# rccohn/AMPIS

Hardware: AMD Instinct MI355X
Metric: images/sec Mask R-CNN R50-FPN @1024x1024 inference (higher is better)
Workload: dtype f32 (convs: f16x3 split-operand MFMA -- 22-bit operands, exact products, fp32 accumulate); 1 GPU; BASELINE configs[1]: R50-FPN inference, batch=8 synthetic 1024x1024 micrographs per GPU, K=2, 1000 proposals/img, TEST.DETECTIONS_PER_IMAGE=200, seeded random-init weights, outputs on the host: boxes, scores, classes and every mask as its COCO compressed-RLE counts string (encoded on the device); batch_per_gpu=8, global_batch=8, parallelism=image-parallel replicas x1, no data-path collective

## Files before the change

ampis_amd/csrc/conv.hip:

```cpp
#include "common.h"
#include <type_traits>

namespace {

typedef float f32x4 __attribute__((ext_vector_type(4)));
typedef float f32x16 __attribute__((ext_vector_type(16)));
typedef _Float16 f16x8 __attribute__((ext_vector_type(8)));
typedef _Float16 f16x2 __attribute__((ext_vector_type(2)));
typedef _Float16 f16x4 __attribute__((ext_vector_type(4)));
typedef unsigned int u32x4 __attribute__((ext_vector_type(4)));
constexpr float LO_SCALE = 2048.0f;

constexpr int BK = 32;
constexpr int LDS_LD = 36;

struct ConvArgs {
    const float* x;
    const float* w;
    const float* scale;
    const float* shift;
    const float* res;
    const float* mask;
    float* y;
    int B, H, W, Cin;
// ... 169 lines not shown
            } else {
#pragma unroll
                for (int q = 0; q < 4; ++q)
                    if (n + q < a.Cout) o[q] = a.mask[yoff[it] + q] > 0.f ? o[q] : 0.f;
            }
        }
        if (vec) {
            *reinterpret_cast<f32x4*>(a.y + yoff[it]) = o;
        } else {
#pragma unroll
            for (int q = 0; q < 4; ++q)
                if (n + q < a.Cout) a.y[yoff[it] + q] = o[q];
        }
    }
}

template <int MB, int NB>
struct F16x3Frags {
    f16x8 ah[MB], al[MB], bh[NB], bl[NB];
};
template <int MB, int NB>
__device__ __forceinline__ void f16x3_load16(const float* As, const float* Bs, int fo_hi, int fo_lo, F16x3Frags<MB, NB>& f) {
#pragma unroll
    for (int i = 0; i < MB; ++i) {
        f.ah[i] = *reinterpret_cast<const f16x8*>(As + i * 16 * BK + fo_hi);
        f.al[i] = *reinterpret_cast<const f16x8*>(As + i * 16 * BK + fo_lo);
    }
#pragma unroll
    for (int j = 0; j < NB; ++j) {
        f.bh[j] = *reinterpret_cast<const f16x8*>(Bs + j * 16 * BK + fo_hi);
        f.bl[j] = *reinterpret_cast<const f16x8*>(Bs + j * 16 * BK + fo_lo);
    }
}
template <int MB, int NB, bool SWAP = false>
__device__ __forceinline__ void f16x3_mfma16(const F16x3Frags<MB, NB>& f, f32x4 (&acc)[MB][NB], f32x4 (&acx)[MB][NB]) {
#pragma unroll
    for (int i = 0; i < MB; ++i) {
        if (SWAP) {
#pragma unroll
            for (int j = 0; j < NB; ++j) acx[i][j] = __builtin_amdgcn_mfma_f32_16x16x32_f16(f.bh[j], f.al[i], acx[i][j], 0, 0, 0);
#pragma unroll
            for (int j = 0; j < NB; ++j) acx[i][j] = __builtin_amdgcn_mfma_f32_16x16x32_f16(f.bl[j], f.ah[i], acx[i][j], 0, 0, 0);
#pragma unroll
            for (int j = 0; j < NB; ++j) acc[i][j] = __builtin_amdgcn_mfma_f32_16x16x32_f16(f.bh[j], f.ah[i], acc[i][j], 0, 0, 0);
        } else {
#pragma unroll
            for (int j = 0; j < NB; ++j) acx[i][j] = __builtin_amdgcn_mfma_f32_16x16x32_f16(f.al[i], f.bh[j], acx[i][j], 0, 0, 0);
#pragma unroll
            for (int j = 0; j < NB; ++j) acx[i][j] = __builtin_amdgcn_mfma_f32_16x16x32_f16(f.ah[i], f.bl[j], acx[i][j], 0, 0, 0);
#pragma unroll
            for (int j = 0; j < NB; ++j) acc[i][j] = __builtin_amdgcn_mfma_f32_16x16x32_f16(f.ah[i], f.bh[j], acc[i][j], 0, 0, 0);
        }
    }
}
template <int MB, int NB>
__device__ __forceinline__ void f16x3_step16(const float* As, const float* Bs, int fo_hi, int fo_lo, f32x4 (&acc)[MB][NB], f32x4 (&acx)[MB][NB]) {
    F16x3Frags<MB, NB> f;
    f16x3_load16<MB, NB>(As, Bs, fo_hi, fo_lo, f);
    f16x3_mfma16<MB, NB>(f, acc, acx);
}

template <int WTM, int WTN, bool SPATIAL, bool CHECK>
__device__ __forceinline__ void conv_epilogue_rows(const ConvArgs& a, float* stage, int lane, int mw0, int nw0);
template <int WTM, int WTN, bool SPATIAL, bool CHECK>
__device__ __forceinline__ void conv_epilogue_rows8(const ConvArgs& a, float* stage, int lane, int mw0, int nw0);

template <int WTM, int WTN, int MT, int NT, bool SPATIAL, bool CHECK = false>
__device__ __forceinline__ void conv_epilogue_fast(const ConvArgs& a, f32x16 (&acc)[MT][NT], float* lds, int wave, int lane,
                                                   int mw0, int nw0) {
    const int l31 = lane & 31, lh = lane >> 5;
    constexpr int SLD = WTN + 4;
    float* stage = lds + wave * (WTM * SLD);
#pragma unroll
    for (int i = 0; i < MT; ++i)
#pragma unroll
        for (int j = 0; j < NT; ++j)
#pragma unroll
            for (int e = 0; e < 16; ++e)
                stage[(i * 32 + (e & 3) + 8 * (e >> 2) + 4 * lh) * SLD + j * 32 + l31] = acc[i][j][e];
    if (a.y_split && !a.mask && a.out_mode == 0) conv_epilogue_rows8<WTM, WTN, SPATIAL, CHECK>(a, stage, lane, mw0, nw0);
    else conv_epilogue_rows<WTM, WTN, SPATIAL, CHECK>(a, stage, lane, mw0, nw0);
}

template <int WTM, int WTN, int MT, int NT, bool SPATIAL, bool CHECK = false>
__device__ __forceinline__ void conv_epilogue_fast16(const ConvArgs& a, f32x4 (&acc)[MT][NT], float* lds, int wave, int lane,
                                                     int mw0, int nw0) {
    const int l15 = lane & 15, lq = lane >> 4;
    constexpr int SLD = WTN + 4;
    float* stage = lds + wave * (WTM * SLD);
#pragma unroll
    for (int i = 0; i < MT; ++i)
#pragma unroll
        for (int j = 0; j < NT; ++j)
#pragma unroll
            for (int e = 0; e < 4; ++e)
                stage[(i * 16 + 4 * lq + e) * SLD + j * 16 + l15] = acc[i][j][e];
    if (a.y_split && !a.mask && a.out_mode == 0) conv_epilogue_rows8<WTM, WTN, SPATIAL, CHECK>(a, stage, lane, mw0, nw0);
    else conv_epilogue_rows<WTM, WTN, SPATIAL, CHECK>(a, stage, lane, mw0, nw0);
}

template <int WTM, int WTN, bool SPATIAL, bool CHECK>
__device__ __forceinline__ void conv_epilogue_rows8(const ConvArgs& a, float* stage, int lane, int mw0, int nw0) {
    constexpr int SLD = WTN + 4;
    constexpr int L8R = WTN / 8;
    constexpr int RPI = 64 / L8R;
    constexpr int NIT = WTM / RPI;
// ... 1072 lines not shown
            STAMP_T(t2);
            f16x3_load16<MB, NB>(As0 + cur * TILE_FLOATS, Bs0 + cur * TILE_FLOATS, fo16_hi, fo16_lo, fr);
            __builtin_amdgcn_sched_barrier(0);
            STAMP_T(t3);
            if (step + 2 < a.nsteps) stage(nxt);
            __builtin_amdgcn_sched_barrier(0);
            STAMP_T(t4);
            STAMP_ADD(0, t0, t1); STAMP_ADD(3, t1, t2); STAMP_ADD(2, t2, t3); STAMP_ADD(1, t3, t4);
            advance();
        }
        f16x3_mfma16<MB, NB, true>(fr, acc, acx);
    }
#ifdef AMP_STAMP
    if (wave == 0 && lane == 0) {
        atomicAdd(&g_stamp_clk[0], __builtin_amdgcn_s_memtime() - st_mt0);
        atomicAdd(&g_stamp_clk[1], __builtin_amdgcn_s_memrealtime() - st_rt0);
    }
    st_acc[4] = clock64() - st_begin;
    st_acc[5] = st_begin - st_entry;
    const long long st_loop_end = clock64();
#endif
    __syncthreads();
#ifdef AMP_STAMP
    st_acc[7] = clock64() - st_loop_end;
#endif
    const bool scaled_in = a.out_scale != 1.0f;

#pragma unroll
    for (int i = 0; i < MB; ++i)
#pragma unroll
        for (int j = 0; j < NB; ++j)
#pragma unroll
            for (int e = 0; e < 4; ++e) {
                acc[i][j][e] = __fadd_rn(acc[i][j][e], __fmul_rn(acx[i][j][e], 1.0f / LO_SCALE));
                if (scaled_in) acc[i][j][e] *= a.out_scale;
            }
    if constexpr (BM == 128 && BN == 256 && EPI == 3) {
        if (NBP == 1 && a.out_mode == 3) conv_epilogue_predict(a, acc, lds, wave, lane, m0, n0, ppf);
        else conv_epilogue_rpn<NBP>(a, acc, lds, wave, lane, m0, n0);
        return;
    }
    if (a.y_split && (!a.mask || a.mask_split) && (a.out_mode == 0 || (EPI == 2 && a.out_mode == 1 && !a.mask && a.res_mode == 0)) && (a.res_mode == 0 || a.res_split) && a.direct_epi)
        conv_epilogue_direct<EPI == 2, true>(a, acc, lane, m0 + wm * WTM, n0 + wn * WTN);
    else
        conv_epilogue_swapped<WTM, WTN, EPI == 2, true>(a, acc, lds, wave, lane, m0 + wm * WTM, n0 + wn * WTN);
#ifdef AMP_STAMP
    st_acc[6] = clock64() - st_loop_end;
    if (lane == 0)
        for (int q = 0; q < 8; ++q) atomicAdd(&g_stamp[wave * 8 + q], (unsigned long long)st_acc[q]);
#endif
}


__global__ __launch_bounds__(512, 1) void mask_tail_kernel(const ConvArgs a, const unsigned int x_bytes, const unsigned int w_bytes) {
    constexpr int BM = 128, BN = 256, NW = 8, GA = 2, GB = 4, NDMA = GA + GB, NTAP = 4;
    constexpr int TILE_FLOATS = (BM + BN) * BK;
    __shared__ __attribute__((aligned(16))) float lds[3 * TILE_FLOATS + 4 * BM + 2 * 256 + 4 + NTAP * BN];
    float* red = lds + 3 * TILE_FLOATS;
    float* wps = red + 4 * BM;
    float* pbs = wps + 2 * 256;
    float* dbias = pbs + 4;
    const int tid = threadIdx.x, lane = tid & 63;
    const int wave = __builtin_amdgcn_readfirstlane(tid >> 6);
    const int wm = wave >> 2, wn = wave & 3;
    const int l15 = lane & 15, lq = lane >> 4;
    const int m0 = amp::xcd_remap(blockIdx.x, a.nblk) * BM;
    const __amdgpu_buffer_rsrc_t rsrc_x = __builtin_amdgcn_make_buffer_rsrc(const_cast<float*>(a.x), 0, x_bytes, 0x00020000);
    const __amdgpu_buffer_rsrc_t rsrc_w = __builtin_amdgcn_make_buffer_rsrc(const_cast<float*>(a.w), 0, w_bytes, 0x00020000);
    const int srow = lane >> 3, spos = lane & 7;
    unsigned int a_voff[GA], b_voff[GB];
#pragma unroll
    for (int g = 0; g < GA; ++g) {
        const int r = wave * (BM / NW) + 8 * g + srow;
        const int m = m0 + r;
        a_voff[g] = (m < a.M) ? (unsigned int)(((size_t)m * a.Cin + 4 * (spos ^ ((r >> 1) & 7))) * 4) : OOB_VOFF;
    }
#pragma unroll
    for (int g = 0; g < GB; ++g) {
        const int r = wave * (BN / NW) + 8 * g + srow;
        const int n = (r & ~63) + swap_channel(r & 63);
        b_voff[g] = (unsigned int)(((size_t)n * a.K + 4 * (spos ^ ((r >> 1) & 7))) * 4);
    }
    const int csteps = a.Cin / BK;
    const int total = NTAP * csteps;
    const int tap_bytes = BN * a.K * 4;
    int s_cs = 0, s_tap = 0;
    auto stage = [&](int buf) {
        float* As = lds + buf * TILE_FLOATS;
        float* Bs = As + BM * BK;
        const int a_soff = s_cs * (BK * 4);
        const int b_soff = s_tap * tap_bytes + s_cs * (BK * 4);
#pragma unroll
        for (int g = 0; g < GA; ++g)
            __builtin_amdgcn_raw_ptr_buffer_load_lds(rsrc_x, (__attribute__((address_space(3))) void*)(As + (wave * (BM / NW) + 8 * g) * BK), 16, (int)a_voff[g], a_soff, 0, 0);
#pragma unroll
        for (int g = 0; g < GB; ++g)
            __builtin_amdgcn_raw_ptr_buffer_load_lds(rsrc_w, (__attribute__((address_space(3))) void*)(Bs + (wave * (BN / NW) + 8 * g) * BK), 16, (int)b_voff[g], b_soff, 0, 0);
        if (++s_cs == csteps) { s_cs = 0; ++s_tap; }
    };
    f32x4 acc[4][4], acx[4][4];
    auto zero_acc = [&]() {
#pragma unroll
        for (int i = 0; i < 4; ++i)
#pragma unroll
            for (int j = 0; j < 4; ++j)
#pragma unroll
                for (int e = 0; e < 4; ++e) { acc[i][j][e] = 0.f; acx[i][j][e] = 0.f; }
    };
    zero_acc();
    const int fo16_hi = 4 * (lq ^ (l15 >> 1)), fo16_lo = 4 * ((4 + lq) ^ (l15 >> 1));
    stage(0);
    stage(1);
    const int mw0 = m0 + wm * 64;
    const unsigned int b_first = fastdiv(min((unsigned int)m0, (unsigned int)(a.M - 1)), a.div_howo_mul, a.div_howo_shr);
    {
        const unsigned int b_last = fastdiv(min((unsigned int)(m0 + BM - 1), (unsigned int)(a.M - 1)), a.div_howo_mul, a.div_howo_shr);
        const int slot = tid >> 8, col = tid & 255;
        int c = a.pred_cls[slot ? b_last : b_first];
        c = (c >= 0 && c < a.pred_K) ? c : 0;
        wps[tid] = a.pred_w[(size_t)c * 256 + col];
        if (col == 0) pbs[slot] = a.pred_b[c];
        dbias[tid] = a.shift ? a.shift[tid] : 0.f;
        dbias[512 + tid] = a.shift ? a.shift[512 + tid] : 0.f;
    }
    bool bad = false;
    auto partial_sums = [&](int tap) {
        f32x4 bias[4];
#pragma unroll
        for (int j = 0; j < 4; ++j) bias[j] = *reinterpret_cast<const f32x4*>(dbias + tap * BN + wn * 64 + 32 * (j >> 1) + 8 * lq + 4 * (j & 1));
#pragma unroll
        for (int i = 0; i < 4; ++i) {
            const unsigned int m = min((unsigned int)(mw0 + i * 16 + l15), (unsigned int)(a.M - 1));
            const unsigned int b = fastdiv(m, a.div_howo_mul, a.div_howo_shr);
            const float* wrow = wps + ((b == b_first) ? 0 : 256) + wn * 64 + 8 * lq;
            float sj[4];
#pragma unroll
            for (int j = 0; j < 4; ++j) {
                const f32x4 wp = *reinterpret_cast<const f32x4*>(wrow + 32 * (j >> 1) + 4 * (j & 1));
                float sg = 0.f;
#pragma unroll
                for (int e = 0; e < 4; ++e) {
                    const float v = __fadd_rn(acc[i][j][e], __fmul_rn(acx[i][j][e], 1.0f / LO_SCALE));
                    bad = bad || !(fabsf(v) <= 3.0e38f);
                    const float o = fmaxf(__fadd_rn(v, bias[j][e]), 0.f);
                    sg = __fadd_rn(sg, __fmul_rn(o, wp[e]));
                }
                sj[j] = sg;
            }
            float u0 = __fadd_rn(sj[0], sj[2]), u1 = __fadd_rn(sj[1], sj[3]);
            u0 = __fadd_rn(u0, __shfl_xor(u0, 32)); u1 = __fadd_rn(u1, __shfl_xor(u1, 32));
            u0 = __fadd_rn(u0, __shfl_xor(u0, 16)); u1 = __fadd_rn(u1, __shfl_xor(u1, 16));
            const float sres = __fadd_rn(u0, u1);
            if (lq == 0) red[wn * BM + wm * 64 + i * 16 + l15] = sres;
        }
    };
    auto finish_rows = [&](int tap) {
        const int rl = wm * 64 + lane;
        const int m = m0 + rl;
        if (m < a.M) {
            const unsigned int b = fastdiv((unsigned int)m, a.div_howo_mul, a.div_howo_shr);
            const unsigned int rem = (unsigned int)m - b * (unsigned int)(a.Ho * a.Wo);
            const unsigned int oy = fastdiv(rem, a.div_wo_mul, a.div_wo_shr);
            const unsigned int ox = rem - oy * (unsigned int)a.Wo;
            float x = __fadd_rn(__fadd_rn(__fadd_rn(red[rl], red[BM + rl]), red[2 * BM + rl]), red[3 * BM + rl]);
            x = __fadd_rn(x, pbs[(b == b_first) ? 0 : 1]);
            const float p = __fdiv_rn(1.0f, __fadd_rn(1.0f, expf(-x)));
            a.prob[((size_t)b * 2 * a.Ho + 2 * oy + (tap >> 1)) * (2 * a.Wo) + 2 * ox + (tap & 1)] = p;
        }
    };
    int cur = 0, nxt = 2, c_cs = 0, c_tap = 0;
    auto open_step = [&](int step) {
        if (step + 1 < total) __builtin_amdgcn_s_waitcnt(0x0070 | NDMA);
        else __builtin_amdgcn_s_waitcnt(0x0070);
        asm volatile("" ::: "memory");
        __builtin_amdgcn_s_barrier();
        asm volatile("" ::: "memory");
    };
    auto advance = [&]() {
        cur = (cur == 2) ? 0 : cur + 1;
        nxt = (nxt == 2) ? 0 : nxt + 1;
        if (++c_cs == csteps) { c_cs = 0; ++c_tap; }
    };
    F16x3Frags<4, 4> fr;
    const float* As0 = lds + (wm * 64 + l15) * BK;
    const float* Bs0 = lds + BM * BK + (wn * 64 + l15) * BK;
    if (wave < NW / 2) {
        for (int step = 0; step < total; ++step) {
            open_step(step);
            if (c_cs == 0 && c_tap > 0 && wn == 0) finish_rows(c_tap - 1);
            f16x3_load16<4, 4>(As0 + cur * TILE_FLOATS, Bs0 + cur * TILE_FLOATS, fo16_hi, fo16_lo, fr);
            __builtin_amdgcn_sched_barrier(0);
            if (step + 2 < total) stage(nxt);
            __builtin_amdgcn_sched_barrier(0);
            __builtin_amdgcn_s_barrier();
            __builtin_amdgcn_s_setprio(1);
            f16x3_mfma16<4, 4, true>(fr, acc, acx);
            __builtin_amdgcn_s_setprio(0);
            __builtin_amdgcn_sched_barrier(0);
            if (c_cs == csteps - 1) { partial_sums(c_tap); zero_acc(); }
            advance();
        }
    } else {
        for (int step = 0; step < total; ++step) {
            open_step(step);
            __builtin_amdgcn_s_setprio(1);
            if (step > 0) f16x3_mfma16<4, 4, true>(fr, acc, acx);
            __builtin_amdgcn_s_setprio(0);
            __builtin_amdgcn_sched_barrier(0);
            const bool tap_done = c_cs == 0 && c_tap > 0;
            if (tap_done) { partial_sums(c_tap - 1); zero_acc(); __builtin_amdgcn_s_waitcnt(0xc07f); }
            __builtin_amdgcn_s_barrier();
            if (tap_done && wn == 0) finish_rows(c_tap - 1);
            f16x3_load16<4, 4>(As0 + cur * TILE_FLOATS, Bs0 + cur * TILE_FLOATS, fo16_hi, fo16_lo, fr);
            __builtin_amdgcn_sched_barrier(0);
            if (step + 2 < total) stage(nxt);
            __builtin_amdgcn_sched_barrier(0);
            advance();
        }
        f16x3_mfma16<4, 4, true>(fr, acc, acx);
        partial_sums(NTAP - 1);
    }
    __syncthreads();
    if (wn == 0) finish_rows(NTAP - 1);
    if (bad) atomicOr(a.range_flag, 1);
}

template <bool SPATIAL>
__global__ __launch_bounds__(512, 1) void conv1x1_nloop_kernel(const ConvArgs a, const unsigned int x_bytes, const unsigned int w_bytes, const int NT) {
    constexpr int BM = 128, BN = 256, NW = 8, GA = 2, GB = 4, NDMA = GA + GB, NST = 16;
    constexpr int TILE_FLOATS = (BM + BN) * BK;
    constexpr int NT_MAX = 8;
    __shared__ __attribute__((aligned(16))) float lds[3 * TILE_FLOATS + 2 * NT_MAX * BN];
    float* lsc = lds + 3 * TILE_FLOATS;
    float* lsh = lsc + NT_MAX * BN;
    const int tid = threadIdx.x, lane = tid & 63;
    const int wave = __builtin_amdgcn_readfirstlane(tid >> 6);
    const int wm = wave >> 2, wn = wave & 3;
    const int l15 = lane & 15, lq = lane >> 4;
    const int ngrp = a.ntn / NT;
    const int wg = amp::xcd_remap(blockIdx.x, a.nblk);
    const int grp = wg % ngrp;
    const int m0 = (wg / ngrp) * BM;
    const int n_first = grp * NT * BN;
    const bool full = m0 + BM <= a.M;
    const __amdgpu_buffer_rsrc_t rsrc_x = __builtin_amdgcn_make_buffer_rsrc(const_cast<float*>(a.x), 0, x_bytes, 0x00020000);
    const __amdgpu_buffer_rsrc_t rsrc_w = __builtin_amdgcn_make_buffer_rsrc(const_cast<float*>(a.w), 0, w_bytes, 0x00020000);
    const int srow = lane >> 3, spos = lane & 7;
    unsigned int a_voff[GA], b_voff[GB];
#pragma unroll
    for (int g = 0; g < GA; ++g) {
        const int r = wave * (BM / NW) + 8 * g + srow;
        const int m = m0 + r;
        a_voff[g] = OOB_VOFF;
        if (m < a.M) {
            const unsigned int b = fastdiv((unsigned int)m, a.div_howo_mul, a.div_howo_shr);
            const unsigned int rem = (unsigned int)m - b * (unsigned int)(a.Ho * a.Wo);
            const unsigned int oy = fastdiv(rem, a.div_wo_mul, a.div_wo_shr);
            const unsigned int ox = rem - oy * (unsigned int)a.Wo;
            a_voff[g] = (unsigned int)((((size_t)(b * a.H + oy * a.stride) * a.W + ox * a.stride) * a.Cin + 4 * (spos ^ ((r >> 1) & 7))) * 4);
        }
    }
#pragma unroll
    for (int g = 0; g < GB; ++g) {
        const int r = wave * (BN / NW) + 8 * g + srow;
        const int n = n_first + (r & ~63) + swap_channel(r & 63);
        b_voff[g] = (unsigned int)(((size_t)n * a.K + 4 * (spos ^ ((r >> 1) & 7))) * 4);
    }
    const int csteps = a.Cin / BK;
    const int total = NT * csteps;
    const int tile_bytes = BN * a.K * 4;
    int s_cs = 0, s_tile = 0;
    auto stage = [&](int buf) {
        float* As = lds + buf * TILE_FLOATS;
        float* Bs = As + BM * BK;
        const int a_soff = s_cs * (BK * 4);
        const int b_soff = s_tile * tile_bytes + s_cs * (BK * 4);
#pragma unroll
// ... 1014 lines not shown
    switch (epi) {
        case 1: AMP_TIMED_LAUNCH((conv_f16x3_kernel<BN, 1, false, true>), dim3(a.nblk), dim3(NT_), 0, st, a, xb, wb); break;
        case 2: AMP_TIMED_LAUNCH((conv_f16x3_kernel<BN, 2, false, true>), dim3(a.nblk), dim3(NT_), 0, st, a, xb, wb); break;
        default: AMP_TIMED_LAUNCH((conv_f16x3_kernel<BN, 0, false, true>), dim3(a.nblk), dim3(NT_), 0, st, a, xb, wb);
    }
}

template <int BN>
void launch_f16x3(const ConvArgs& a, int epi, hipStream_t st, unsigned int xb, unsigned int wb) {
    if (a.in_scale != 1.0f) { launch_f16x3_scaled<BN>(a, epi, st, xb, wb); return; }
    constexpr int NT_ = (BN == 256) ? 512 : 256;
    switch (epi) {
        case 1: AMP_TIMED_LAUNCH((conv_f16x3_kernel<BN, 1>), dim3(a.nblk), dim3(NT_), 0, st, a, xb, wb); break;
        case 2: AMP_TIMED_LAUNCH((conv_f16x3_kernel<BN, 2>), dim3(a.nblk), dim3(NT_), 0, st, a, xb, wb); break;
        default: AMP_TIMED_LAUNCH((conv_f16x3_kernel<BN, 0>), dim3(a.nblk), dim3(NT_), 0, st, a, xb, wb);
    }
}

void set_fastdiv(unsigned int d, unsigned int* mul, int* shr) {
    int l = 0;
    while ((1ull << l) < d) ++l;
    *shr = 29 + l;
    *mul = (unsigned int)(((1ull << *shr) + d - 1) / d);
}

}

struct ConvSwitches {
    int f16x3_bn256 = 1;
    int short_k = getenv("AMP_NO_SHORT_K") ? 0 : 1;
    int tall64 = getenv("AMP_TALL64") ? atoi(getenv("AMP_TALL64")) : 1;
    int split_ring = getenv("AMP_SPLIT_RING") ? atoi(getenv("AMP_SPLIT_RING")) : 1;
    int korder = getenv("AMP_KORDER") ? atoi(getenv("AMP_KORDER")) : 0;
    int patch256 = getenv("AMP_PATCH256") ? atoi(getenv("AMP_PATCH256")) : 0;
    int nloop = getenv("AMP_NLOOP") ? atoi(getenv("AMP_NLOOP")) : 0;
    int mask_tail_loop = getenv("AMP_NO_MASK_TAIL_LOOP") ? 0 : 1;
    int patch_conv = getenv("AMP_NO_PATCH_CONV") ? 0 : 1;
    int stagger = getenv("AMP_STAGGER") ? atoi(getenv("AMP_STAGGER")) : 1;
    int generic_epi = 0;
    int ablate = 0;
};
static ConvSwitches g_sw;
extern "C" void amp_debug_set_f16x3_bn256(int v) { g_sw.f16x3_bn256 = v; }
extern "C" void amp_debug_set_short_k(int v) { g_sw.short_k = v; }
extern "C" void amp_debug_set_tall64(int v) { g_sw.tall64 = v; }
extern "C" void amp_debug_set_split_ring(int v) { g_sw.split_ring = v; }
extern "C" void amp_debug_set_korder(int v) { g_sw.korder = v; }
extern "C" void amp_debug_set_patch256(int v) { g_sw.patch256 = v; }
extern "C" void amp_debug_set_nloop(int v) { g_sw.nloop = v; }
extern "C" void amp_debug_set_mask_tail_loop(int v) { g_sw.mask_tail_loop = v; }
extern "C" void amp_debug_set_patch_conv(int v) { g_sw.patch_conv = v; }
extern "C" void amp_debug_set_conv_generic_epilogue(int on) { g_sw.generic_epi = on; }
extern "C" void amp_debug_set_conv_ablate(int mode) { g_sw.ablate = mode; }
constexpr int WIDE_NSTEPS = 64;
constexpr int SHORT_K_STEPS = 16;
#ifdef AMP_STAMP
extern "C" int amp_debug_read_stamps(unsigned long long* out) {
    if (hipMemcpyFromSymbol(out, HIP_SYMBOL(g_stamp), sizeof(unsigned long long) * 64) != hipSuccess) return -1;
    unsigned long long z[64] = {0};
    return hipMemcpyToSymbol(HIP_SYMBOL(g_stamp), z, sizeof(z)) == hipSuccess ? 0 : -1;
}
extern "C" int amp_debug_read_stamp_clock(unsigned long long* out) {
    if (hipMemcpyFromSymbol(out, HIP_SYMBOL(g_stamp_clk), sizeof(unsigned long long) * 2) != hipSuccess) return -1;
    unsigned long long z[2] = {0, 0};
    return hipMemcpyToSymbol(HIP_SYMBOL(g_stamp_clk), z, sizeof(z)) == hipSuccess ? 0 : -1;
}
#endif

static int conv_impl(amp_ctx* ctx, const amp_conv_desc* d, int groups, const float* x, const float* w, const float* scale,
                     const float* shift, const float* res, const float* mask, float* y) {
    return amp::conv_run(ctx, d, groups, x, w, nullptr, 0, scale, shift, res, mask, y);
}

int amp::weight_jobs_run(amp_ctx* ctx, const amp::WeightJob* jobs_dev, const void* chunks_dev, int nchunks) {
    if (nchunks <= 0) return AMP_OK;
    hipLaunchKernelGGL(weight_jobs_kernel, dim3((unsigned)nchunks), dim3(256), 0, ctx->stream, jobs_dev, reinterpret_cast<const uint2*>(chunks_dev));
    AMP_HIP_CHECK(hipGetLastError());
    return AMP_OK;
}

extern "C" int amp_dgrad_weights_split(amp_ctx* ctx, const float* w, const float* scale, int Cout, int KH, int KW, int Cin, float* wt_split) {
    AMP_REQUIRE(ctx && w && wt_split && Cout > 0 && KH > 0 && KW > 0 && Cin > 0 && Cout % 32 == 0, "amp_dgrad_weights_split: bad argument (Cout %% 32 != 0?)");
    amp::WeightJob job{w, scale, reinterpret_cast<unsigned int*>(wt_split), Cout, KH, KW, Cin, (Cout % 64 == 0 && Cin % 64 == 0) ? 2 : 1};
    std::vector<unsigned int> ch;
    if (job.transpose == 2) {
        const size_t ntiles = (size_t)KH * KW * (Cout / 64) * (Cin / 64);
        for (size_t t = 0; t < ntiles; ++t) { ch.push_back(0u); ch.push_back((unsigned int)t); }
    } else {
        const size_t npairs = (size_t)Cout * KH * KW * Cin / 2;
        for (size_t p0 = 0; p0 < npairs; p0 += 8192) { ch.push_back(0u); ch.push_back((unsigned int)p0); }
    }
    amp::WeightJob* d_job = nullptr;
    unsigned int* d_ch = nullptr;
    AMP_HIP_CHECK(hipMalloc(&d_job, sizeof(job)));
    if (hipMalloc(&d_ch, ch.size() * sizeof(unsigned int)) != hipSuccess) { (void)hipFree(d_job); AMP_REQUIRE(false, "amp_dgrad_weights_split: out of device memory"); }
    int st = AMP_OK;
    if (hipMemcpy(d_job, &job, sizeof(job), hipMemcpyHostToDevice) != hipSuccess ||
        hipMemcpy(d_ch, ch.data(), ch.size() * sizeof(unsigned int), hipMemcpyHostToDevice) != hipSuccess) st = AMP_ERR_HIP;
    if (st == AMP_OK) st = amp::weight_jobs_run(ctx, d_job, d_ch, (int)(ch.size() / 2));
    if (st == AMP_OK && hipStreamSynchronize(ctx->stream) != hipSuccess) st = AMP_ERR_HIP;
    (void)hipFree(d_job);
    (void)hipFree(d_ch);
    return st;
}

extern "C" int amp_split_weights(amp_ctx* ctx, const float* w, long long rows, int K, float* w_split) {
    AMP_REQUIRE(ctx && w && w_split && rows > 0 && K > 0 && K % 32 == 0, "amp_split_weights: bad argument (K %% 32 != 0?)");
    hipLaunchKernelGGL(split_weights_kernel, dim3(2048), dim3(256), 0, ctx->stream, w, (size_t)rows, K, reinterpret_cast<unsigned int*>(w_split));
    AMP_HIP_CHECK(hipGetLastError());
    return AMP_OK;
}

namespace {
__global__ void unsplit_rows_kernel(const unsigned int* __restrict__ in, size_t rows, int C, float* __restrict__ out) {
    const size_t total = rows * (size_t)(C / 2);
    for (size_t i = (size_t)blockIdx.x * blockDim.x + threadIdx.x; i < total; i += (size_t)gridDim.x * blockDim.x) {
        const size_t r = i / (C / 2);
        const int kp = (int)(i - r * (C / 2));
// ... 552 lines not shown
    AMP_REQUIRE(!(fuse && rpn), "conv: the fused RPN epilogue needs a split input, Cout = 256, ReLU and the ring kernel");
    ConvPlan p;
    AMP_TRY_STATUS(conv_plan({ctx->conv_mode, *d, groups, fmt, in_shift, force_f32, res != nullptr, mask != nullptr, scale != nullptr,
                              fuse ? 1 : (rpn ? 2 : 0), rpn ? rpn->ld : 0}, g_sw, &p));
    const double MN = (double)p.M * d->Cout;
    const double in_rows = (d->KH == 1 && d->KW == 1) ? (double)p.M : (double)d->B * d->H * d->W;
    const double out_vals = p.out_mode == 3 ? (double)p.M * 4.0 : p.out_mode == 4 ? (double)p.M * 16.0 * p.rpn_nbp : MN;
    const double res_vals = !res ? 0.0 : (d->res_mode == 2 ? MN / 4.0 : MN);
    amp_prof_rec* rec = prof_open(ctx, 2.0 * MN * (double)d->KH * (double)d->KW * (double)p.cpg,
                                  4.0 * (in_rows * d->Cin + (double)d->Cout * p.K + out_vals + res_vals + (mask ? MN : 0.0)),
                                  p.M, d->Cout, d->KH * d->KW * p.cpg, p.dominant ? 0 : 1);
    amp::ProfLaunchScope timed(rec ? rec->e0 : nullptr, rec ? rec->e1 : nullptr);
    if (p.f16x3 && !w_split) {
        if (ctx->split_bytes < p.w_bytes) {
            AMP_HIP_CHECK(hipStreamSynchronize(ctx->stream));
            if (ctx->split_scratch) AMP_HIP_CHECK(hipFree(ctx->split_scratch));
            ctx->split_scratch = nullptr; ctx->split_bytes = 0;
            AMP_HIP_CHECK(hipMalloc(&ctx->split_scratch, p.w_bytes));
            ctx->split_bytes = p.w_bytes;
        }
        hipLaunchKernelGGL(split_weights_kernel, dim3(2048), dim3(256), 0, ctx->stream, w, (size_t)d->Cout, p.K,
                           reinterpret_cast<unsigned int*>(ctx->split_scratch));
        w_split = ctx->split_scratch;
    }
    ConvArgs a;
    a.x = x; a.w = p.f16x3 ? w_split : w; a.scale = scale; a.shift = shift; a.res = res; a.mask = mask; a.y = y;
    a.B = d->B; a.H = d->H; a.W = d->W; a.Cin = d->Cin; a.Cout = d->Cout;
    a.KH = d->KH; a.KW = d->KW; a.stride = d->stride; a.pad = d->pad;
    a.Ho = p.Ho; a.Wo = p.Wo; a.M = p.M; a.K = p.K; a.nsteps = p.nsteps;
    a.grouped = groups > 1; a.cin_win = p.cin_win;
    a.relu = d->relu; a.res_mode = d->res_mode; a.out_mode = p.out_mode;
    a.ntn = p.ntn; a.nblk = p.nblk; a.stagger = p.stagger; a.korder = p.korder; a.direct_epi = 1;
    a.in_scale = (in_shift != 0) ? ldexpf(1.0f, in_shift) : 1.0f;
    a.out_scale = (in_shift != 0) ? ldexpf(1.0f, -in_shift) : 1.0f;
    a.y_split = p.y_split; a.res_split = (fmt & 4) ? 1 : 0; a.mask_split = (fmt & 8) ? 1 : 0;
    a.range_flag = ctx->d_conv_flag;
    a.pred_w = fuse ? fuse->pred_w : nullptr; a.pred_b = fuse ? fuse->pred_b : nullptr; a.pred_cls = fuse ? fuse->cls : nullptr;
    a.pred_K = fuse ? fuse->K : 0; a.prob = fuse ? fuse->prob : nullptr;
    a.rpn_w = rpn ? rpn->w_split : nullptr; a.rpn_b = rpn ? rpn->bias : nullptr; a.rpn_pred = rpn ? rpn->pred : nullptr;
    set_fastdiv((unsigned int)(a.Ho * a.Wo), &a.div_howo_mul, &a.div_howo_shr);
    set_fastdiv((unsigned int)a.Wo, &a.div_wo_mul, &a.div_wo_shr);
    const unsigned int xb = (unsigned int)p.x_bytes, wb = (unsigned int)p.w_bytes;
    hipStream_t st = ctx->stream;
    using amp::ConvKernel;
    switch (p.kernel) {
        case ConvKernel::C64_PATCH_DIAG: AMP_TIMED_LAUNCH(conv3x3_c64_kernel<true>, dim3(a.nblk), dim3(256), 0, st, a, xb, wb, p.tiles_x, p.tiles_y, Fuse3Args()); break;
        case ConvKernel::C64_PATCH: AMP_TIMED_LAUNCH(conv3x3_c64_kernel<false>, dim3(a.nblk), dim3(256), 0, st, a, xb, wb, p.tiles_x, p.tiles_y, Fuse3Args()); break;
        case ConvKernel::PATCH256:
            if (p.epi == 5) AMP_TIMED_LAUNCH(conv3x3_patch_kernel<5>, dim3(a.nblk), dim3(512), 0, st, a, xb, wb, p.tiles_x, p.tiles_y);
            else if (p.epi == 4) AMP_TIMED_LAUNCH(conv3x3_patch_kernel<4>, dim3(a.nblk), dim3(512), 0, st, a, xb, wb, p.tiles_x, p.tiles_y);
            else if (p.epi == 3) AMP_TIMED_LAUNCH(conv3x3_patch_kernel<3>, dim3(a.nblk), dim3(512), 0, st, a, xb, wb, p.tiles_x, p.tiles_y);
            else AMP_TIMED_LAUNCH(conv3x3_patch_kernel<1>, dim3(a.nblk), dim3(512), 0, st, a, xb, wb, p.tiles_x, p.tiles_y);
            break;
        case ConvKernel::MASK_TAIL: AMP_TIMED_LAUNCH(mask_tail_kernel, dim3(a.nblk), dim3(512), 0, st, a, xb, wb); break;
        case ConvKernel::SPLIT_128x256: launch_split<128, 256>(a, p.epi, st, xb, wb); break;
        case ConvKernel::SPLIT_SHORT_128x128: launch_split_short(a, p.epi, st, xb, wb); break;
        case ConvKernel::NLOOP_SCATTER: AMP_TIMED_LAUNCH(conv1x1_nloop_kernel<true>, dim3(a.nblk), dim3(512), 0, st, a, xb, wb, p.nloop_nt); break;
        case ConvKernel::NLOOP: AMP_TIMED_LAUNCH(conv1x1_nloop_kernel<false>, dim3(a.nblk), dim3(512), 0, st, a, xb, wb, p.nloop_nt); break;
        case ConvKernel::SPLIT_256x128: launch_split<256, 128>(a, p.epi, st, xb, wb); break;
        case ConvKernel::SPLIT_TALL64: launch_split_tall64(a, st, xb, wb); break;
        case ConvKernel::F16X3S_256: launch_f16x3s<256>(a, p.epi, st, xb, wb); break;
        case ConvKernel::F16X3S_128: launch_f16x3s<128>(a, p.epi, st, xb, wb); break;
        case ConvKernel::F16X3S_G32: launch_f16x3s_g32(a, p.epi, st, xb, wb); break;
        case ConvKernel::F16X3S_64: launch_f16x3s<64>(a, p.epi, st, xb, wb); break;
        case ConvKernel::F16X3_STEM: launch_f16x3_stem(a, p.epi, st, xb, wb); break;
        case ConvKernel::F16X3_64: launch_f16x3<64>(a, p.epi, st, xb, wb); break;
        case ConvKernel::F16X3_256: launch_f16x3<256>(a, p.epi, st, xb, wb); break;
        case ConvKernel::F16X3_128: launch_f16x3<128>(a, p.epi, st, xb, wb); break;
        case ConvKernel::GLDS_STEM: launch_glds<64, true>(a, p.epi, st, xb, wb); break;
        case ConvKernel::GLDS_128: launch_glds<128, false>(a, p.epi, st, xb, wb); break;
        case ConvKernel::GLDS_64: launch_glds<64, false>(a, p.epi, st, xb, wb); break;
        case ConvKernel::MFMA_128:
            if (g_sw.ablate == 1) AMP_TIMED_LAUNCH((conv_mfma_kernel<128, 128, 1>), dim3(a.nblk), dim3(256), 0, st, a);
            else if (g_sw.ablate == 2) AMP_TIMED_LAUNCH((conv_mfma_kernel<128, 128, 2>), dim3(a.nblk), dim3(256), 0, st, a);
            else if (g_sw.ablate == 3) AMP_TIMED_LAUNCH((conv_mfma_kernel<128, 128, 3>), dim3(a.nblk), dim3(256), 0, st, a);
            else AMP_TIMED_LAUNCH((conv_mfma_kernel<128, 128, 0>), dim3(a.nblk), dim3(256), 0, st, a);
            break;
        case ConvKernel::MFMA_64: AMP_TIMED_LAUNCH((conv_mfma_kernel<128, 64>), dim3(a.nblk), dim3(256), 0, st, a); break;
        case ConvKernel::COUNT: break;
    }
    AMP_HIP_CHECK(hipGetLastError());
    return AMP_OK;
}

struct amp_debug_conv_plan_out { int kernel, epi, ntn, nblk, stagger, dominant, tiles_x, tiles_y, nloop_nt, rpn_nbp; };
extern "C" int amp_debug_conv_plan(const int* in, const int* sw, amp_debug_conv_plan_out* out) {
    AMP_REQUIRE(in && out, "amp_debug_conv_plan: null argument");
    ConvPlanIn pi;
    pi.mode = in[0];
    pi.d.B = in[1]; pi.d.H = in[2]; pi.d.W = in[3]; pi.d.Cin = in[4]; pi.d.Cout = in[5]; pi.d.KH = in[6]; pi.d.KW = in[7]; pi.d.stride = in[8]; pi.d.pad = in[9];
    pi.d.relu = in[10]; pi.d.res_mode = in[11]; pi.d.out_mode = in[12];
    pi.groups = in[13]; pi.fmt = in[14]; pi.in_shift = in[15]; pi.force_f32 = in[16];
    pi.res = in[17] != 0; pi.mask = in[18] != 0; pi.scale = in[19] != 0; pi.fuse = in[20]; pi.rpn_ld = in[21];
    ConvSwitches s = g_sw;
    if (sw) {
        s.f16x3_bn256 = sw[0]; s.short_k = sw[1]; s.tall64 = sw[2]; s.split_ring = sw[3]; s.korder = sw[4]; s.patch256 = sw[5]; s.nloop = sw[6];
        s.mask_tail_loop = sw[7]; s.patch_conv = sw[8]; s.stagger = sw[9]; s.generic_epi = sw[10]; s.ablate = sw[11];
    }
    ConvPlan p;
    AMP_TRY_STATUS(conv_plan(pi, s, &p));
    *out = {(int)p.kernel, p.epi, p.ntn, p.nblk, p.stagger, p.dominant ? 1 : 0, p.tiles_x, p.tiles_y, p.nloop_nt, p.rpn_nbp};
    return AMP_OK;
}
extern "C" const char* amp_debug_conv_kernel_name(int kernel) {
    static const char* const names[] = {"C64_PATCH", "C64_PATCH_DIAG", "PATCH256", "MASK_TAIL", "SPLIT_128x256", "SPLIT_SHORT_128x128", "SPLIT_256x128", "SPLIT_TALL64",
                                        "NLOOP", "NLOOP_SCATTER", "F16X3S_256", "F16X3S_128", "F16X3S_64", "F16X3S_G32", "F16X3_STEM", "F16X3_256", "F16X3_128", "F16X3_64",
                                        "GLDS_STEM", "GLDS_128", "GLDS_64", "MFMA_128", "MFMA_64"};
// ... 40 lines not shown
```

Before: 496.9 images/s.

## Overlap mask-tail per-tap reduction with last-step MFMAs and drop accumulator zeroing

New measurement: 499.7 images/s, median of 6. About the same (+0.6%).

```diff
diff --git a/ampis_amd/csrc/conv.hip b/ampis_amd/csrc/conv.hip
--- a/ampis_amd/csrc/conv.hip
+++ b/ampis_amd/csrc/conv.hip
@@ -245,6 +245,16 @@
             for (int j = 0; j < NB; ++j) acc[i][j] = __builtin_amdgcn_mfma_f32_16x16x32_f16(f.ah[i], f.bh[j], acc[i][j], 0, 0, 0);
         }
     }
+}
+template <int MB, int NB, bool ZERO>
+__device__ __forceinline__ void f16x3_mfma16_row(const F16x3Frags<MB, NB>& f, int i, f32x4 (&acc)[NB], f32x4 (&acx)[NB]) {
+    const f32x4 z = {0.f, 0.f, 0.f, 0.f};
+#pragma unroll
+    for (int j = 0; j < NB; ++j) acx[j] = __builtin_amdgcn_mfma_f32_16x16x32_f16(f.bh[j], f.al[i], ZERO ? z : acx[j], 0, 0, 0);
+#pragma unroll
+    for (int j = 0; j < NB; ++j) acx[j] = __builtin_amdgcn_mfma_f32_16x16x32_f16(f.bl[j], f.ah[i], acx[j], 0, 0, 0);
+#pragma unroll
+    for (int j = 0; j < NB; ++j) acc[j] = __builtin_amdgcn_mfma_f32_16x16x32_f16(f.bh[j], f.ah[i], ZERO ? z : acc[j], 0, 0, 0);
 }
 template <int MB, int NB>
 __device__ __forceinline__ void f16x3_step16(const float* As, const float* Bs, int fo_hi, int fo_lo, f32x4 (&acc)[MB][NB], f32x4 (&acx)[MB][NB]) {
@@ -1423,6 +1433,10 @@
 }
 
 
+#ifdef AMP_STAMP
+__device__ unsigned long long g_stamp_mt[8 * 8];
+#endif
+template <bool OVL>
 __global__ __launch_bounds__(512, 1) void mask_tail_kernel(const ConvArgs a, const unsigned int x_bytes, const unsigned int w_bytes) {
     constexpr int BM = 128, BN = 256, NW = 8, GA = 2, GB = 4, NDMA = GA + GB, NTAP = 4;
     constexpr int TILE_FLOATS = (BM + BN) * BK;
@@ -1431,6 +1445,10 @@
     float* wps = red + 4 * BM;
     float* pbs = wps + 2 * 256;
     float* dbias = pbs + 4;
+#ifdef AMP_STAMP
+    const long long st_entry = clock64();
+    long long st_acc[8] = {0, 0, 0, 0, 0, 0, 0, 0};
+#endif
     const int tid = threadIdx.x, lane = tid & 63;
     const int wave = __builtin_amdgcn_readfirstlane(tid >> 6);
     const int wm = wave >> 2, wn = wave & 3;
@@ -1478,7 +1496,7 @@
 #pragma unroll
                 for (int e = 0; e < 4; ++e) { acc[i][j][e] = 0.f; acx[i][j][e] = 0.f; }
     };
-    zero_acc();
+    if constexpr (!OVL) zero_acc();
     const int fo16_hi = 4 * (lq ^ (l15 >> 1)), fo16_lo = 4 * ((4 + lq) ^ (l15 >> 1));
     stage(0);
     stage(1);
@@ -1495,35 +1513,60 @@
         dbias[512 + tid] = a.shift ? a.shift[512 + tid] : 0.f;
     }
     bool bad = false;
-    auto partial_sums = [&](int tap) {
+    F16x3Frags<4, 4> fr;
+    auto load_bias = [&](int tap, f32x4 (&bias)[4]) __attribute__((always_inline)) {
+#pragma unroll
+        for (int j = 0; j < 4; ++j) bias[j] = *reinterpret_cast<const f32x4*>(dbias + tap * BN + wn * 64 + 32 * (j >> 1) + 8 * lq + 4 * (j & 1));
+    };
+    auto row_sums = [&](int i, const f32x4 (&bias)[4]) __attribute__((always_inline)) {
+        const unsigned int m = min((unsigned int)(mw0 + i * 16 + l15), (unsigned int)(a.M - 1));
+        const unsigned int b = fastdiv(m, a.div_howo_mul, a.div_howo_shr);
+        const float* wrow = wps + ((b == b_first) ? 0 : 256) + wn * 64 + 8 * lq;
+        float sj[4];
+#pragma unroll
+        for (int j = 0; j < 4; ++j) {
+            const f32x4 wp = *reinterpret_cast<const f32x4*>(wrow + 32 * (j >> 1) + 4 * (j & 1));
+            float sg = 0.f;
+#pragma unroll
+            for (int e = 0; e < 4; ++e) {
+                const float v = __fadd_rn(acc[i][j][e], __fmul_rn(acx[i][j][e], 1.0f / LO_SCALE));
+                bad = bad || !(fabsf(v) <= 3.0e38f);
+                const float o = fmaxf(__fadd_rn(v, bias[j][e]), 0.f);
+                sg = __fadd_rn(sg, __fmul_rn(o, wp[e]));
+            }
+            sj[j] = sg;
+        }
+        float u0 = __fadd_rn(sj[0], sj[2]), u1 = __fadd_rn(sj[1], sj[3]);
+        u0 = __fadd_rn(u0, __shfl_xor(u0, 32)); u1 = __fadd_rn(u1, __shfl_xor(u1, 32));
+        u0 = __fadd_rn(u0, __shfl_xor(u0, 16)); u1 = __fadd_rn(u1, __shfl_xor(u1, 16));
+        const float sres = __fadd_rn(u0, u1);
+        if (lq == 0) red[wn * BM + wm * 64 + i * 16 + l15] = sres;
+    };
+    auto partial_sums = [&](int tap) __attribute__((always_inline)) {
         f32x4 bias[4];
-#pragma unroll
-        for (int j = 0; j < 4; ++j) bias[j] = *reinterpret_cast<const f32x4*>(dbias + tap * BN + wn * 64 + 32 * (j >> 1) + 8 * lq + 4 * (j & 1));
-#pragma unroll
-        for (int i = 0; i < 4; ++i) {
-            const unsigned int m = min((unsigned int)(mw0 + i * 16 + l15), (unsigned int)(a.M - 1));
-            const unsigned int b = fastdiv(m, a.div_howo_mul, a.div_howo_shr);
-            const float* wrow = wps + ((b == b_first) ? 0 : 256) + wn * 64 + 8 * lq;
-            float sj[4];
-#pragma unroll
-            for (int j = 0; j < 4; ++j) {
-                const f32x4 wp = *reinterpret_cast<const f32x4*>(wrow + 32 * (j >> 1) + 4 * (j & 1));
-                float sg = 0.f;
-#pragma unroll
-                for (int e = 0; e < 4; ++e) {
-                    const float v = __fadd_rn(acc[i][j][e], __fmul_rn(acx[i][j][e], 1.0f / LO_SCALE));
-                    bad = bad || !(fabsf(v) <= 3.0e38f);
-                    const float o = fmaxf(__fadd_rn(v, bias[j][e]), 0.f);
-                    sg = __fadd_rn(sg, __fmul_rn(o, wp[e]));
-                }
-                sj[j] = sg;
-            }
-            float u0 = __fadd_rn(sj[0], sj[2]), u1 = __fadd_rn(sj[1], sj[3]);
-            u0 = __fadd_rn(u0, __shfl_xor(u0, 32)); u1 = __fadd_rn(u1, __shfl_xor(u1, 32));
-            u0 = __fadd_rn(u0, __shfl_xor(u0, 16)); u1 = __fadd_rn(u1, __shfl_xor(u1, 16));
-            const float sres = __fadd_rn(u0, u1);
-            if (lq == 0) red[wn * BM + wm * 64 + i * 16 + l15] = sres;
-        }
+        load_bias(tap, bias);
+#pragma unroll
+        for (int i = 0; i < 4; ++i) row_sums(i, bias);
+    };
+    auto tap_last = [&](int tap) __attribute__((always_inline)) {
+        f16x3_mfma16_row<4, 4, false>(fr, 0, acc[0], acx[0]);
+#pragma unroll
+        for (int i = 1; i < 4; ++i) {
+            __builtin_amdgcn_sched_barrier(0);
+            f16x3_mfma16_row<4, 4, false>(fr, i, acc[i], acx[i]);
+            f32x4 bias[4];
+            load_bias(tap, bias);
+            row_sums(i - 1, bias);
+        }
+        __builtin_amdgcn_sched_barrier(0);
+        __builtin_amdgcn_s_setprio(0);
+        f32x4 bias[4];
+        load_bias(tap, bias);
+        row_sums(3, bias);
+    };
+    auto mfma_first = [&]() __attribute__((always_inline)) {
+#pragma unroll
+        for (int i = 0; i < 4; ++i) f16x3_mfma16_row<4, 4, true>(fr, i, acc[i], acx[i]);
     };
     auto finish_rows = [&](int tap) {
         const int rl = wm * 64 + lane;
@@ -1552,48 +1595,155 @@
         nxt = (nxt == 2) ? 0 : nxt + 1;
         if (++c_cs == csteps) { c_cs = 0; ++c_tap; }
     };
-    F16x3Frags<4, 4> fr;
     const float* As0 = lds + (wm * 64 + l15) * BK;
     const float* Bs0 = lds + BM * BK + (wn * 64 + l15) * BK;
+#ifdef AMP_STAMP
+    const long long st_begin = clock64();
+#endif
+    if constexpr (OVL) {
+        int step = 0;
+        auto next = [&]() __attribute__((always_inline)) { advance(); ++step; };
+        if (wave < NW / 2) {
+            auto early_step = [&](int kind, int tap) __attribute__((always_inline)) {
+                STAMP_T(t0);
+                open_step(step);
+                STAMP_T(t1);
+                if (kind == 0 && tap > 0 && wn == 0) finish_rows(tap - 1);
+                STAMP_T(t2);
+                f16x3_load16<4, 4>(As0 + cur * TILE_FLOATS, Bs0 + cur * TILE_FLOATS, fo16_hi, fo16_lo, fr);
+                __builtin_amdgcn_sched_barrier(0);
+                if (step + 2 < total) stage(nxt);
+                __builtin_amdgcn_sched_barrier(0);
+                STAMP_T(t3);
+                __builtin_amdgcn_s_barrier();
+                STAMP_T(t4);
+                __builtin_amdgcn_s_setprio(1);
+                if (kind == 0) mfma_first();
+                else if (kind == 1) f16x3_mfma16<4, 4, true>(fr, acc, acx);
+                else tap_last(tap);
+                __builtin_amdgcn_s_setprio(0);
+                __builtin_amdgcn_sched_barrier(0);
+#ifdef AMP_STAMP
+                const long long t5 = clock64();
+                if (step == 0) st_acc[0] = t1 - st_entry;
+                if (kind == 2) st_acc[3] += t5 - t4;
+#endif
+                STAMP_ADD(1, t0, t1); STAMP_ADD(4, t1, t2); STAMP_ADD(2, t3, t4);
+                next();
+            };
+            for (int tap = 0; tap < NTAP; ++tap) {
+                early_step(0, tap);
+                for (int cs = 2; cs < csteps; ++cs) early_step(1, tap);
+                early_step(2, tap);
+            }
+        } else {
+            auto late_step = [&](int kind, int tap) __attribute__((always_inline)) {
+                STAMP_T(t0);
+                open_step(step);
+                STAMP_T(t1);
+                __builtin_amdgcn_s_setprio(1);
+                if (kind == 0) mfma_first();
+                else if (kind == 1) f16x3_mfma16<4, 4, true>(fr, acc, acx);
+                else if (kind == 2) { tap_last(tap); __builtin_amdgcn_s_waitcnt(0xc07f); }
+                __builtin_amdgcn_s_setprio(0);
+                __builtin_amdgcn_sched_barrier(0);
+                STAMP_T(t2);
+                __builtin_amdgcn_s_barrier();
+                STAMP_T(t3);
+                if (kind == 2 && wn == 0) finish_rows(tap);
+                STAMP_T(t4);
+                f16x3_load16<4, 4>(As0 + cur * TILE_FLOATS, Bs0 + cur * TILE_FLOATS, fo16_hi, fo16_lo, fr);
+                __builtin_amdgcn_sched_barrier(0);
+                if (step + 2 < total) stage(nxt);
+                __builtin_amdgcn_sched_barrier(0);
+#ifdef AMP_STAMP
+                if (step == 0) st_acc[0] = t1 - st_entry;
+                if (kind == 2) st_acc[3] += t2 - t1;
+#endif
+                STAMP_ADD(1, t0, t1); STAMP_ADD(2, t2, t3); STAMP_ADD(4, t3, t4);
+                next();
+            };
+            late_step(-1, 0);
+            for (int tap = 0; tap < NTAP - 1; ++tap) {
+                late_step(0, tap);
+                for (int cs = 2; cs < csteps; ++cs) late_step(1, tap);
+                late_step(2, tap);
+            }
+            late_step(0, NTAP - 1);
+            for (int cs = 2; cs < csteps; ++cs) late_step(1, NTAP - 1);
+            __builtin_amdgcn_s_setprio(1);
+            tap_last(NTAP - 1);
+        }
+    } else
     if (wave < NW / 2) {
         for (int step = 0; step < total; ++step) {
+            STAMP_T(t0);
             open_step(step);
+            STAMP_T(t1);
             if (c_cs == 0 && c_tap > 0 && wn == 0) finish_rows(c_tap - 1);
+            STAMP_T(t2);
             f16x3_load16<4, 4>(As0 + cur * TILE_FLOATS, Bs0 + cur * TILE_FLOATS, fo16_hi, fo16_lo, fr);
             __builtin_amdgcn_sched_barrier(0);
             if (step + 2 < total) stage(nxt);
             __builtin_amdgcn_sched_barrier(0);
+            STAMP_T(t3);
             __builtin_amdgcn_s_barrier();
+            STAMP_T(t4);
             __builtin_amdgcn_s_setprio(1);
             f16x3_mfma16<4, 4, true>(fr, acc, acx);
             __builtin_amdgcn_s_setprio(0);
             __builtin_amdgcn_sched_barrier(0);
             if (c_cs == csteps - 1) { partial_sums(c_tap); zero_acc(); }
+#ifdef AMP_STAMP
+            const long long t5 = clock64();
+            if (step == 0) st_acc[0] = t1 - st_entry;
+            if (c_cs == csteps - 1) st_acc[3] += t5 - t4;
+#endif
+            STAMP_ADD(1, t0, t1); STAMP_ADD(4, t1, t2); STAMP_ADD(2, t3, t4);
             advance();
         }
     } else {
         for (int step = 0; step < total; ++step) {
+            STAMP_T(t0);
             open_step(step);
+            STAMP_T(t1);
             __builtin_amdgcn_s_setprio(1);
             if (step > 0) f16x3_mfma16<4, 4, true>(fr, acc, acx);
             __builtin_amdgcn_s_setprio(0);
             __builtin_amdgcn_sched_barrier(0);
             const bool tap_done = c_cs == 0 && c_tap > 0;
             if (tap_done) { partial_sums(c_tap - 1); zero_acc(); __builtin_amdgcn_s_waitcnt(0xc07f); }
+            STAMP_T(t2);
             __builtin_amdgcn_s_barrier();
+            STAMP_T(t3);
             if (tap_done && wn == 0) finish_rows(c_tap - 1);
+            STAMP_T(t4);
             f16x3_load16<4, 4>(As0 + cur * TILE_FLOATS, Bs0 + cur * TILE_FLOATS, fo16_hi, fo16_lo, fr);
             __builtin_amdgcn_sched_barrier(0);
             if (step + 2 < total) stage(nxt);
             __builtin_amdgcn_sched_barrier(0);
+#ifdef AMP_STAMP
+            if (step == 0) st_acc[0] = t1 - st_entry;
+            if (tap_done) st_acc[3] += t2 - t1;
+#endif
+            STAMP_ADD(1, t0, t1); STAMP_ADD(2, t2, t3); STAMP_ADD(4, t3, t4);
             advance();
         }
         f16x3_mfma16<4, 4, true>(fr, acc, acx);
         partial_sums(NTAP - 1);
     }
+#ifdef AMP_STAMP
+    const long long st_loop_end = clock64();
+#endif
     __syncthreads();
     if (wn == 0) finish_rows(NTAP - 1);
     if (bad) atomicOr(a.range_flag, 1);
+#ifdef AMP_STAMP
+    const long long st_exit = clock64();
+    st_acc[5] = st_loop_end - st_begin; st_acc[6] = st_exit - st_loop_end; st_acc[7] = st_exit - st_entry;
+    if (lane == 0)
+        for (int q = 0; q < 8; ++q) atomicAdd(&g_stamp_mt[wave * 8 + q], (unsigned long long)st_acc[q]);
+#endif
 }
 
 template <bool SPATIAL>
@@ -2714,6 +2864,8 @@
 extern "C" void amp_debug_set_patch_conv(int v) { g_sw.patch_conv = v; }
 extern "C" void amp_debug_set_conv_generic_epilogue(int on) { g_sw.generic_epi = on; }
 extern "C" void amp_debug_set_conv_ablate(int mode) { g_sw.ablate = mode; }
+static int g_mask_tail_v1 = getenv("AMP_MASK_TAIL_V1") ? atoi(getenv("AMP_MASK_TAIL_V1")) : 0;
+extern "C" void amp_debug_set_mask_tail_v1(int v) { g_mask_tail_v1 = v; }
 constexpr int WIDE_NSTEPS = 64;
 constexpr int SHORT_K_STEPS = 16;
 #ifdef AMP_STAMP
@@ -2726,6 +2878,11 @@
     if (hipMemcpyFromSymbol(out, HIP_SYMBOL(g_stamp_clk), sizeof(unsigned long long) * 2) != hipSuccess) return -1;
     unsigned long long z[2] = {0, 0};
     return hipMemcpyToSymbol(HIP_SYMBOL(g_stamp_clk), z, sizeof(z)) == hipSuccess ? 0 : -1;
+}
+extern "C" int amp_debug_read_mask_tail_stamps(unsigned long long* out) {
+    if (hipMemcpyFromSymbol(out, HIP_SYMBOL(g_stamp_mt), sizeof(unsigned long long) * 64) != hipSuccess) return -1;
+    unsigned long long z[64] = {0};
+    return hipMemcpyToSymbol(HIP_SYMBOL(g_stamp_mt), z, sizeof(z)) == hipSuccess ? 0 : -1;
 }
 #endif
 
@@ -3384,7 +3541,10 @@
             else if (p.epi == 3) AMP_TIMED_LAUNCH(conv3x3_patch_kernel<3>, dim3(a.nblk), dim3(512), 0, st, a, xb, wb, p.tiles_x, p.tiles_y);
             else AMP_TIMED_LAUNCH(conv3x3_patch_kernel<1>, dim3(a.nblk), dim3(512), 0, st, a, xb, wb, p.tiles_x, p.tiles_y);
             break;
-        case ConvKernel::MASK_TAIL: AMP_TIMED_LAUNCH(mask_tail_kernel, dim3(a.nblk), dim3(512), 0, st, a, xb, wb); break;
+        case ConvKernel::MASK_TAIL:
+            if (g_mask_tail_v1 || a.Cin < 2 * BK) AMP_TIMED_LAUNCH(mask_tail_kernel<false>, dim3(a.nblk), dim3(512), 0, st, a, xb, wb);
+            else AMP_TIMED_LAUNCH(mask_tail_kernel<true>, dim3(a.nblk), dim3(512), 0, st, a, xb, wb);
+            break;
         case ConvKernel::SPLIT_128x256: launch_split<128, 256>(a, p.epi, st, xb, wb); break;
         case ConvKernel::SPLIT_SHORT_128x128: launch_split_short(a, p.epi, st, xb, wb); break;
         case ConvKernel::NLOOP_SCATTER: AMP_TIMED_LAUNCH(conv1x1_nloop_kernel<true>, dim3(a.nblk), dim3(512), 0, st, a, xb, wb, p.nloop_nt); break;
```
